# planck-epoch/unet-image-segmentation

Measured on AMD Instinct MI355X. Metric: images/sec (train step, 256x256x3), higher is better.
Workload: dtype f32; 1 GPU; configs[1]: 256x256x3 binary U-Net train step (fwd + dice_loss + bwd + AdamW + MeanIoU(2) update, dropout 0.2); network=U_NET separable-conv, filters 64-128-256-512, bneck 1024, global_batch=16, per_gpu_batch=16, seq_len=65536, parallelism=dp1, batchnorm=per-replica

## Files before the change

unet-image-segmentation_amd/csrc/gemm.h:

```cpp
#pragma once
#include "gemm_plan.h"
#include "view.h"

namespace unet {

struct RowsArgs {
    DView a;
    int64_t M;
    int K;
    int uH, uW, uf;
    const float* B;
    int64_t sbk, sbn;
    int N;
    float* C;
    int64_t ldc;
    const float* bias;
    float2* stats;
    int sH, sW, sf;
    const float* z;
    const float* coef;
    float* side;
    const float *bsc, *bsh, *bmu, *brs;
    float* bnpart;
    float ep_rate, ep_inv_keep;
    uint64_t ep_seed;
    int ko;
    const unsigned short* Bx;
};

struct WgradArgs {
    DView a;
    int P;
    int uH, uW, uf;
    DView b;
    int Q;
    int64_t M, mslice;
    float* slab;
    const float* bz;
    const float* bcoef;
    float* colpart;
};

template <int AMODE, bool DROP, int EPI>
int launch_rows(const RowsArgs& a, hipStream_t st, const char* what);
bool rows_vec_ok(const RowsArgs& a, int amode);
int run_wgrad(WgradArgs a, int amode, int bmode, float* out, void* ws, size_t ws_bytes, hipStream_t st,
              const char* what);
size_t wgrad_workspace(int64_t M, int P, int Q);

inline DView plain_view(const float* p, int c) {
    unet_view v{};
    v.mode = UNET_VIEW_PLAIN;
    v.c0 = c;
    v.src0 = p;
    return make_dview(v);
}
inline bool fits_i32(int64_t a, int64_t b) { return a * b < (int64_t(1) << 31); }
inline int check_planes(const unsigned short* p, const char* what) {
    UNET_CHECK_ARG(p && (uintptr_t)p % 16 == 0, "%s must be a 16-B aligned plane set", what);
    return 0;
}

__device__ __forceinline__ int acc_row(int r, int hi) { return (r & 3) + 8 * (r >> 2) + 4 * hi; }

__device__ __forceinline__ void xcd_group_order(int groups, int sibs, int& grp, int& sib) {
    grp = blockIdx.x;
    sib = blockIdx.y;
    if (sibs > 1 && (groups & 7) == 0) {
        const int L = blockIdx.x + blockIdx.y * groups, u = L >> 3;
        grp = (u / sibs) * 8 + (L & 7);
        sib = u % sibs;
    }
}
__device__ __forceinline__ void xcd_group_order_sx(int sibs, int groups, int& sib, int& grp) {
    sib = blockIdx.x;
    grp = blockIdx.y;
    if (sibs > 1 && (groups & 7) == 0) {
        const int L = blockIdx.x + blockIdx.y * sibs, u = L >> 3;
        grp = (u / sibs) * 8 + (L & 7);
        sib = u % sibs;
    }
}

__device__ __forceinline__ int shuffle_tap_off(int c, int W, int f) {
    const int ab = c / f;
    const int co = c - ab * f;
    return (ab >> 1) * (2 * W * f) + (ab & 1) * f + co;
}


#ifdef UNET_LAB_BUILD
#define ROWS_KO(g, bit) (((g).ko & (bit)) != 0)
__device__ __forceinline__ void lab_stagger(int ko) {
    const int n = (ko >> 8) & 255;
    if (n == 0) return;
    const unsigned lin = blockIdx.x + blockIdx.y * gridDim.x, tot = gridDim.x * gridDim.y;
    const bool late = (ko & 0x10000) ? (lin & 1) : (lin >= tot / 2);
    if (late)
        for (int i = 0; i < n; ++i) __builtin_amdgcn_s_sleep(32);
}
#define ROWS_STAGGER(g) lab_stagger((g).ko)
#define ROWS_STAMP(g, i)                                                                       \
    do {                                                                                       \
        if (((g).ko & 0x20000) && threadIdx.x == 0) {                                          \
            const unsigned lin_ = blockIdx.x + blockIdx.y * gridDim.x;                         \
            if (lin_ < 65536) lab_rows_stamps[4 * lin_ + (i)] =                               \
                ((i) == 0 || (i) == 3) ? __builtin_amdgcn_s_memrealtime() : __builtin_amdgcn_s_memtime(); \
        }                                                                                      \
    } while (0)
#else
#define ROWS_KO(g, bit) false
#define ROWS_STAGGER(g) ((void)0)
#define ROWS_STAMP(g, i) ((void)0)
#endif

}
```

unet-image-segmentation_amd/csrc/gemm_wgrad.hip:

```cpp
#include "dispatch.h"
#include "gemm.h"

namespace unet {
namespace {

template <int BP, int BQ, int AMODE, bool ADROP, int BMODE, bool BDROP>
__global__ __launch_bounds__(256) void gemm_wgrad_kernel(WgradArgs g) {
    constexpr int LDA = BP + 4, LDB = BQ + 4;
    constexpr int TM = BP / 64, TN = BQ / 64;
    constexpr int AR = BP / 16, BR = BQ / 16;
    constexpr int AS = 256 / BP, BS = 256 / BQ;
    __shared__ float As[2][BK][LDA];
    __shared__ float Bs[2][BK][LDB];

    const int tid = threadIdx.x, lane = tid & 63, wave = tid >> 6;
    const int wp = wave >> 1, wq = wave & 1;
    const int lo = lane & 31, hi = lane >> 5;
    const int ntp = (g.P + BP - 1) / BP;
    const int p0 = (blockIdx.x % ntp) * BP;
    const int q0 = (blockIdx.x / ntp) * BQ;
    const int64_t mb = (int64_t)blockIdx.y * g.mslice;
    const int64_t me = mb + g.mslice < g.M ? mb + g.mslice : g.M;

    const int ap = tid % BP, amm = tid / BP;
    const int p = p0 + ap;
    const bool pv = p < g.P;
    float asc = 1.f, ash = 0.f;
    int poff = p;
    if constexpr (AMODE == W_BNRELU) {
        if (pv) {
            asc = g.a.sc0[p];
            ash = g.a.sh0[p];
        }
    }
    if constexpr (AMODE == W_UNSHUFFLE) {
        const int ab = p / g.uf;
        const int co = p - ab * g.uf;
        poff = (ab >> 1) * (2 * g.uW * g.uf) + (ab & 1) * g.uf + co;
    }
    const int bq = tid % BQ, bmm = tid / BQ;
    const int q = q0 + bq;
    const bool qv = q < g.Q;
    float bsc = 1.f, bsh = 0.f;
    if constexpr (BMODE == W_BNRELU) {
        if (qv) {
            bsc = g.b.sc0[q];
            bsh = g.b.sh0[q];
        }
    }

    float ra[AR], rb[BR];
    auto load_stage = [&](int64_t k0) {
#pragma unroll
        for (int r = 0; r < AR; ++r) {
            const int64_t m = k0 + amm + AS * r;
            float v = 0.f;
            if (pv && m < me) {
                if constexpr (AMODE == W_UNSHUFFLE) {
                    const int64_t hw = (int64_t)g.uH * g.uW;
                    const int n = (int)(m / hw);
                    const int rem = (int)(m - n * hw);
                    const int i = rem / g.uW, j = rem - (rem / g.uW) * g.uW;
                    v = g.a.src0[(int64_t)((n * 2 * g.uH + 2 * i) * 2 * g.uW + 2 * j) * g.uf + poff];
                } else {
                    v = g.a.src0[m * g.a.c0 + p];
                    if constexpr (AMODE == W_BNRELU) v = bnrelu(v, asc, ash);
                    if constexpr (ADROP) v *= drop_mult(g.a.seed, (uint64_t)m * g.a.C + p, g.a.rate, g.a.inv_keep);
                }
            }
            ra[r] = v;
        }
#pragma unroll
        for (int r = 0; r < BR; ++r) {
            const int64_t m = k0 + bmm + BS * r;
            float v = 0.f;
            if (qv && m < me) {
                v = g.b.src0[m * g.b.c0 + q];
                if constexpr (BMODE == W_BNRELU) v = bnrelu(v, bsc, bsh);
                if constexpr (BDROP) v *= drop_mult(g.b.seed, (uint64_t)m * g.b.C + q, g.b.rate, g.b.inv_keep);
            }
            rb[r] = v;
        }
    };
    auto store_stage = [&](int buf) {
#pragma unroll
        for (int r = 0; r < AR; ++r) As[buf][amm + AS * r][ap] = ra[r];
#pragma unroll
        for (int r = 0; r < BR; ++r) Bs[buf][bmm + BS * r][bq] = rb[r];
    };

    floatx16 acc[TM][TN];
#pragma unroll
    for (int tm = 0; tm < TM; ++tm)
#pragma unroll
        for (int tn = 0; tn < TN; ++tn)
#pragma unroll
            for (int r = 0; r < 16; ++r) acc[tm][tn][r] = 0.f;

    const int nk = (int)((me - mb + BK - 1) / BK);
    if (nk > 0) {
        load_stage(mb);
        store_stage(0);
    }
    __syncthreads();
    for (int kt = 0; kt < nk; ++kt) {
        const int buf = kt & 1;
        if (kt + 1 < nk) load_stage(mb + (int64_t)(kt + 1) * BK);
#pragma unroll
        for (int kk = 0; kk < BK / 2; ++kk) {
            float av[TM], bv[TN];
#pragma unroll
            for (int tm = 0; tm < TM; ++tm) av[tm] = As[buf][2 * kk + hi][wp * (BP / 2) + tm * 32 + lo];
#pragma unroll
            for (int tn = 0; tn < TN; ++tn) bv[tn] = Bs[buf][2 * kk + hi][wq * (BQ / 2) + tn * 32 + lo];
#pragma unroll
            for (int tm = 0; tm < TM; ++tm)
#pragma unroll
                for (int tn = 0; tn < TN; ++tn)
                    acc[tm][tn] = __builtin_amdgcn_mfma_f32_32x32x2f32(av[tm], bv[tn], acc[tm][tn], 0, 0, 0);
        }
        if (kt + 1 < nk) store_stage(buf ^ 1);
        __syncthreads();
    }
    float* slab = g.slab + (int64_t)blockIdx.y * g.P * g.Q;
#pragma unroll
    for (int tm = 0; tm < TM; ++tm)
#pragma unroll
        for (int tn = 0; tn < TN; ++tn) {
            const int qq = q0 + wq * (BQ / 2) + tn * 32 + lo;
            if (qq >= g.Q) continue;
#pragma unroll
            for (int r = 0; r < 16; ++r) {
                const int pp = p0 + wp * (BP / 2) + tm * 32 + acc_row(r, hi);
                if (pp < g.P) slab[(int64_t)pp * g.Q + qq] = acc[tm][tn][r];
            }
        }
}

template <int BP, int BQ, int AMODE, bool ADROP, int BMODE, bool BDROP>
__global__ __launch_bounds__(256, 1) void gemm_wgrad_vec(WgradArgs g) {
    constexpr int LDA = BP + 4, LDB = BQ + 4;
    constexpr int TM = BP / 64, TN = BQ / 64;
    constexpr int PQ = BP / 4, QQ = BQ / 4;
    constexpr int AR = BK * PQ / 256, BR = BK * QQ / 256;
    constexpr int AS = 256 / PQ, BS = 256 / QQ;
    __shared__ __attribute__((aligned(16))) char smem[4 * 2 * BK * (LDA + LDB)];
    float (*As)[BK * LDA] = reinterpret_cast<float (*)[BK * LDA]>(smem);
    float (*Bs)[BK * LDB] = reinterpret_cast<float (*)[BK * LDB]>(smem + 4 * 2 * BK * LDA);

    const int tid = threadIdx.x, lane = tid & 63, wave = tid >> 6;
    const int wp = wave >> 1, wq = wave & 1;
    const int lo = lane & 31, hi = lane >> 5;
    const int ntp = (g.P + BP - 1) / BP;
    int tile, slice;
    xcd_group_order_sx(gridDim.x, gridDim.y, tile, slice);
    const int p0 = (tile % ntp) * BP;
    const int q0 = (tile / ntp) * BQ;
    const int mb = (int)(slice * g.mslice);
    const int me = (int)((mb + g.mslice) < g.M ? (mb + g.mslice) : g.M);

    const int apq = tid % PQ, amm = tid / PQ;
    const int p = p0 + 4 * apq;
    const bool pv = p < g.P;
    float4 asc = f4(1.f), ash = f4(0.f);
    int poff = p;
    if constexpr (AMODE == W_BNRELU) {
        if (pv) {
            asc = ld4(g.a.sc0 + p);
            ash = ld4(g.a.sh0 + p);
        }
    }
    if constexpr (AMODE == W_UNSHUFFLE) {
        const int ab = p / g.uf;
        const int co = p - ab * g.uf;
        poff = (ab >> 1) * (2 * g.uW * g.uf) + (ab & 1) * g.uf + co;
    }
    const int bqq = tid % QQ, bmm = tid / QQ;
    const int q = q0 + 4 * bqq;
    const bool qv = q < g.Q;
    float4 bsc = f4(1.f), bsh = f4(0.f), bmu = f4(0.f), bp_ = f4(0.f), bq_ = f4(0.f);
    if constexpr (BMODE == W_BNRELU || BMODE == W_BNBWD) {
        if (qv) {
            bsc = ld4(g.b.sc0 + q);
            bsh = ld4(g.b.sh0 + q);
        }
    }
    if constexpr (BMODE == W_BNBWD) {
        if (qv) {
            bmu = ld4(g.bcoef + q);
            bp_ = ld4(g.bcoef + g.Q + q);
            bq_ = ld4(g.bcoef + 2 * g.Q + q);
        }
    }

    float4 ra[AR], rb[BR];
    int ur[AMODE == W_UNSHUFFLE ? AR : 1], uj[AMODE == W_UNSHUFFLE ? AR : 1];
    if constexpr (AMODE == W_UNSHUFFLE) {
#pragma unroll
        for (int r = 0; r < AR; ++r) {
            const int m = mb + amm + AS * r;
            ur[r] = m / g.uW;
            uj[r] = m - ur[r] * g.uW;
        }
    }
    auto load_stage = [&](int k0) {
#pragma unroll
        for (int r = 0; r < AR; ++r) {
            const int m = k0 + amm + AS * r;
            float4 v = f4(0.f);
            if (pv && m < me) {
                if constexpr (AMODE == W_UNSHUFFLE) {
                    v = ld4(g.a.src0 + (4 * ur[r] * g.uW + 2 * uj[r]) * g.uf + poff);
                } else {
                    v = ld4(g.a.src0 + (int64_t)m * g.a.c0 + p);
                    if constexpr (AMODE == W_BNRELU) v = bnrelu4(v, asc, ash);
                    if constexpr (ADROP) {
                        const uint64_t i = (uint64_t)m * g.a.C + p;
                        v = mul4(v, drop_mult4(g.a.seed, i, g.a.rate, g.a.inv_keep));
                    }
                }
            }
            ra[r] = v;
        }
#pragma unroll
        for (int r = 0; r < BR; ++r) {
            const int m = k0 + bmm + BS * r;
            float4 v = f4(0.f);
            if (qv && m < me) {
                v = ld4(g.b.src0 + (int64_t)m * g.b.c0 + q);
                if constexpr (BMODE == W_BNRELU) v = bnrelu4(v, bsc, bsh);
                if constexpr (BMODE == W_BNBWD)
                    bn_bwd_dz4(v, ld4(g.bz + (int64_t)m * g.b.c0 + q), bsc, bsh, bmu, bp_, bq_);
                if constexpr (BDROP) {
                    const uint64_t i = (uint64_t)m * g.b.C + q;
                    v = mul4(v, drop_mult4(g.b.seed, i, g.b.rate, g.b.inv_keep));
                }
            }
            rb[r] = v;
        }
        if constexpr (AMODE == W_UNSHUFFLE) {
#pragma unroll
            for (int r = 0; r < AR; ++r) {
                uj[r] += BK;
                while (uj[r] >= g.uW) {
                    uj[r] -= g.uW;
                    ++ur[r];
                }
            }
        }
    };
    const bool csum_on = g.colpart != nullptr && tile < ntp;
    float4 csum = f4(0.f);
    auto store_stage = [&](int buf) {
#pragma unroll
        for (int r = 0; r < AR; ++r) *reinterpret_cast<float4*>(&As[buf][(amm + AS * r) * LDA + 4 * apq]) = ra[r];
#pragma unroll
        for (int r = 0; r < BR; ++r) *reinterpret_cast<float4*>(&Bs[buf][(bmm + BS * r) * LDB + 4 * bqq]) = rb[r];
        if (csum_on) {
#pragma unroll
            for (int r = 0; r < AR; ++r) csum = add4(csum, ra[r]);
        }
    };

    floatx16 acc[TM][TN];
#pragma unroll
    for (int tm = 0; tm < TM; ++tm)
#pragma unroll
        for (int tn = 0; tn < TN; ++tn)
#pragma unroll
            for (int r = 0; r < 16; ++r) acc[tm][tn][r] = 0.f;

    const int nk = (me - mb + BK - 1) / BK;
    if (nk > 0) {
        load_stage(mb);
        store_stage(0);
    }
    __syncthreads();
    for (int kt = 0; kt < nk; ++kt) {
        const int buf = kt & 1;
        if (kt + 1 < nk) load_stage(mb + (kt + 1) * BK);
#pragma unroll
        for (int kk = 0; kk < BK / 2; ++kk) {
            float av[TM], bv[TN];
#pragma unroll
            for (int tm = 0; tm < TM; ++tm) av[tm] = As[buf][(2 * kk + hi) * LDA + wp * (BP / 2) + tm * 32 + lo];
#pragma unroll
            for (int tn = 0; tn < TN; ++tn) bv[tn] = Bs[buf][(2 * kk + hi) * LDB + wq * (BQ / 2) + tn * 32 + lo];
#pragma unroll
            for (int tm = 0; tm < TM; ++tm)
#pragma unroll
                for (int tn = 0; tn < TN; ++tn)
                    acc[tm][tn] = __builtin_amdgcn_mfma_f32_32x32x2f32(av[tm], bv[tn], acc[tm][tn], 0, 0, 0);
        }
        if (kt + 1 < nk) store_stage(buf ^ 1);
        __syncthreads();
    }
    if (csum_on) {
        float4* T = reinterpret_cast<float4*>(&As[0][0]);
        T[tid] = csum;
        __syncthreads();
        if (tid < PQ && pv) {
            float4 t = T[tid];
            for (int j = 1; j < AS; ++j) t = add4(t, T[j * PQ + tid]);
            st4(g.colpart + (int64_t)slice * g.P + p, t);
        }
    }
    float* slab = g.slab + (int64_t)slice * g.P * g.Q;
#pragma unroll
    for (int tm = 0; tm < TM; ++tm)
#pragma unroll
        for (int tn = 0; tn < TN; ++tn) {
            const int qq = q0 + wq * (BQ / 2) + tn * 32 + lo;
            if (qq >= g.Q) continue;
#pragma unroll
            for (int r = 0; r < 16; ++r) {
                const int pp = p0 + wp * (BP / 2) + tm * 32 + acc_row(r, hi);
                if (pp < g.P) slab[(int64_t)pp * g.Q + qq] = acc[tm][tn][r];
            }
        }
}

template <int AMODE, bool ADROP, int BMODE, bool BDROP>
void launch_wgrad_t(const WgradArgs& a, const WgradPlan& w, hipStream_t st) {
    dim3 grid((unsigned)w.tiles, (unsigned)w.S);
    const unsigned pad = (unsigned)lab_knob("UNET_WGRAD_LDSPAD", 0);
    const bool vec = a.P % 4 == 0 && a.Q % 4 == 0 && (AMODE != W_UNSHUFFLE || a.uf % 4 == 0) &&
                     (AMODE == W_UNSHUFFLE || a.a.c0 % 4 == 0) && a.b.c0 % 4 == 0 &&
                     ((uintptr_t)a.a.src0 | (uintptr_t)a.b.src0) % 16 == 0;
    const bool vk = vec || BMODE == W_BNBWD;
    with_int<128, 64>(w.bp, [&](auto BP) {
        with_int<128, 64>(w.bq, [&](auto BQ) {
            if (vk) gemm_wgrad_vec<BP(), BQ(), AMODE, ADROP, BMODE, BDROP><<<grid, 256, pad, st>>>(a);
            else if constexpr (BMODE != W_BNBWD)
                gemm_wgrad_kernel<BP(), BQ(), AMODE, ADROP, BMODE, BDROP><<<grid, 256, pad, st>>>(a);
        });
    });
}

}

int run_wgrad(WgradArgs a, int amode, int bmode, float* out, void* ws, size_t ws_bytes, hipStream_t st,
              const char* what) {
    WgradPlan w = wgrad_plan(a.M, a.P, a.Q);
    const size_t need = (size_t)w.S * a.P * a.Q * sizeof(float);
    UNET_CHECK_ARG(ws && ws_bytes >= need, "%s: workspace %zu < %zu", what, ws_bytes, need);
    a.mslice = w.mslice;
    a.slab = static_cast<float*>(ws);
    const bool ad = a.a.rate > 0.f, bd = a.b.rate > 0.f;
    if (amode == W_PLAIN && bmode == W_PLAIN) {
        launch_wgrad_t<W_PLAIN, false, W_PLAIN, false>(a, w, st);
    } else if (amode == W_UNSHUFFLE && (bmode == W_BNRELU || bmode == W_PLAIN)) {
        with_int<W_BNRELU, W_PLAIN>(bmode, [&](auto BM) {
            with_bool(bd, [&](auto BD) { launch_wgrad_t<W_UNSHUFFLE, false, BM(), BD()>(a, w, st); });
        });
    } else if (amode == W_BNRELU && bmode == W_PLAIN) {
        with_bool(ad, [&](auto AD) { launch_wgrad_t<W_BNRELU, AD(), W_PLAIN, false>(a, w, st); });
    } else {
        UNET_CHECK_ARG(false, "%s: unsupported wgrad operand modes %d/%d", what, amode, bmode);
    }
    UNET_CHECK_LAUNCH(what);
    return reduce_slabs(a.slab, w.S, (int64_t)a.P * a.Q, out, (int64_t)a.P * a.Q, (int64_t)a.P * a.Q, st);
}

size_t wgrad_workspace(int64_t M, int P, int Q) {
    WgradPlan w = wgrad_plan(M, P, Q);
    return align_up((size_t)w.S * P * Q * sizeof(float), 256);
}

int head_wgrad(const unet_view* x, int64_t M, const float* dlogit, int ncls, float* dkernel, void* ws, size_t ws_bytes,
               hipStream_t st) {
    WgradArgs a{};
    a.a = make_dview(*x);
    a.P = x->c0;
    a.b = plain_view(dlogit, ncls);
    a.Q = ncls;
    a.M = M;
    return run_wgrad(a, x->mode == UNET_VIEW_BNRELU ? W_BNRELU : W_PLAIN, W_PLAIN, dkernel, ws, ws_bytes, st,
                     "unet_head_bwd(filter)");
}
size_t head_wgrad_workspace(int64_t M, int cin, int ncls) { return wgrad_workspace(M, cin, ncls); }

}
```

Before: 1660 images/sec.

## Defer B-side BN-ReLU/dropout to store stage and cut unshuffle index registers in wgrad

For the unshuffle A-mode wgrad kernel with BN-ReLU or dropout on B, the per-channel scale/shift now live in LDS and are applied at store time instead of being held in registers across the loop. The unshuffle row/column tracking is reworked into wave-uniform per-row column counters, and the epilogue indices are recomputed from an opaque copy of tid. These changes aim to lower VGPR pressure in the vec wgrad kernel. One variant also gets extra dynamic LDS padding to cap occupancy at a fixed LDS size, which deliberately limits co-resident blocks.

```diff
diff --git a/unet-image-segmentation_amd/csrc/gemm.h b/unet-image-segmentation_amd/csrc/gemm.h
--- a/unet-image-segmentation_amd/csrc/gemm.h
+++ b/unet-image-segmentation_amd/csrc/gemm.h
@@ -61,6 +61,11 @@
     return 0;
 }
 
+constexpr int kSimdRegs = 512;
+constexpr int kMainSmallRegs = 80;
+constexpr int kMainSmallLds = 16384;
+constexpr unsigned kSideCap3Lds = 45056;
+
 __device__ __forceinline__ int acc_row(int r, int hi) { return (r & 3) + 8 * (r >> 2) + 4 * hi; }
 
 __device__ __forceinline__ void xcd_group_order(int groups, int sibs, int& grp, int& sib) {
diff --git a/unet-image-segmentation_amd/csrc/gemm_wgrad.hip b/unet-image-segmentation_amd/csrc/gemm_wgrad.hip
--- a/unet-image-segmentation_amd/csrc/gemm_wgrad.hip
+++ b/unet-image-segmentation_amd/csrc/gemm_wgrad.hip
@@ -144,9 +144,12 @@
     constexpr int PQ = BP / 4, QQ = BQ / 4;
     constexpr int AR = BK * PQ / 256, BR = BK * QQ / 256;
     constexpr int AS = 256 / PQ, BS = 256 / QQ;
-    __shared__ __attribute__((aligned(16))) char smem[4 * 2 * BK * (LDA + LDB)];
+    constexpr bool LATEB = AMODE == W_UNSHUFFLE && (BMODE == W_BNRELU || BDROP);
+    constexpr int STAGE_BYTES = 4 * 2 * BK * (LDA + LDB);
+    __shared__ __attribute__((aligned(16))) char smem[STAGE_BYTES + (LATEB ? 8 * BQ : 0)];
     float (*As)[BK * LDA] = reinterpret_cast<float (*)[BK * LDA]>(smem);
     float (*Bs)[BK * LDB] = reinterpret_cast<float (*)[BK * LDB]>(smem + 4 * 2 * BK * LDA);
+    float* bview = reinterpret_cast<float*>(smem + (LATEB ? STAGE_BYTES : 0));
 
     const int tid = threadIdx.x, lane = tid & 63, wave = tid >> 6;
     const int wp = wave >> 1, wq = wave & 1;
@@ -179,11 +182,19 @@
     const int q = q0 + 4 * bqq;
     const bool qv = q < g.Q;
     float4 bsc = f4(1.f), bsh = f4(0.f), bmu = f4(0.f), bp_ = f4(0.f), bq_ = f4(0.f);
-    if constexpr (BMODE == W_BNRELU || BMODE == W_BNBWD) {
+    if constexpr ((BMODE == W_BNRELU || BMODE == W_BNBWD) && !LATEB) {
         if (qv) {
             bsc = ld4(g.b.sc0 + q);
             bsh = ld4(g.b.sh0 + q);
         }
+    }
+    if constexpr (LATEB && BMODE == W_BNRELU) {
+        if (tid < BQ) {
+            const bool v = q0 + tid < g.Q;
+            bview[tid] = v ? g.b.sc0[q0 + tid] : 1.f;
+            bview[BQ + tid] = v ? g.b.sh0[q0 + tid] : 0.f;
+        }
+        __syncthreads();
     }
     if constexpr (BMODE == W_BNBWD) {
         if (qv) {
@@ -194,14 +205,15 @@
     }
 
     float4 ra[AR], rb[BR];
-    int ur[AMODE == W_UNSHUFFLE ? AR : 1], uj[AMODE == W_UNSHUFFLE ? AR : 1];
+    constexpr int RW = 64 / PQ;
+    const int wrow = __builtin_amdgcn_readfirstlane(wave) * RW;
+    const int asub = amm - wrow;
+    int uj[AMODE == W_UNSHUFFLE ? AR : 1][RW];
     if constexpr (AMODE == W_UNSHUFFLE) {
 #pragma unroll
-        for (int r = 0; r < AR; ++r) {
-            const int m = mb + amm + AS * r;
-            ur[r] = m / g.uW;
-            uj[r] = m - ur[r] * g.uW;
-        }
+        for (int r = 0; r < AR; ++r)
+#pragma unroll
+            for (int k = 0; k < RW; ++k) uj[r][k] = (mb + wrow + AS * r + k) % g.uW;
     }
     auto load_stage = [&](int k0) {
 #pragma unroll
@@ -210,7 +222,10 @@
             float4 v = f4(0.f);
             if (pv && m < me) {
                 if constexpr (AMODE == W_UNSHUFFLE) {
-                    v = ld4(g.a.src0 + (4 * ur[r] * g.uW + 2 * uj[r]) * g.uf + poff);
+                    int off = (4 * (k0 + wrow + AS * r) - 2 * uj[r][0]) * g.uf;
+#pragma unroll
+                    for (int k = 1; k < RW; ++k) off = asub == k ? (4 * (k0 + wrow + AS * r + k) - 2 * uj[r][k]) * g.uf : off;
+                    v = ld4(g.a.src0 + off + poff);
                 } else {
                     v = ld4(g.a.src0 + (int64_t)m * g.a.c0 + p);
                     if constexpr (AMODE == W_BNRELU) v = bnrelu4(v, asc, ash);
@@ -228,32 +243,52 @@
             float4 v = f4(0.f);
             if (qv && m < me) {
                 v = ld4(g.b.src0 + (int64_t)m * g.b.c0 + q);
-                if constexpr (BMODE == W_BNRELU) v = bnrelu4(v, bsc, bsh);
+                if constexpr (BMODE == W_BNRELU && !LATEB) v = bnrelu4(v, bsc, bsh);
                 if constexpr (BMODE == W_BNBWD)
                     bn_bwd_dz4(v, ld4(g.bz + (int64_t)m * g.b.c0 + q), bsc, bsh, bmu, bp_, bq_);
+                if constexpr (BDROP && !LATEB) {
+                    const uint64_t i = (uint64_t)m * g.b.C + q;
+                    v = mul4(v, drop_mult4(g.b.seed, i, g.b.rate, g.b.inv_keep));
+                }
+            }
+            rb[r] = v;
+        }
+        if constexpr (AMODE == W_UNSHUFFLE) {
+#pragma unroll
+            for (int r = 0; r < AR; ++r)
+#pragma unroll
+                for (int k = 0; k < RW; ++k) {
+                    uj[r][k] += BK;
+                    while (uj[r][k] >= g.uW) uj[r][k] -= g.uW;
+                }
+        }
+    };
+    const bool csum_on = g.colpart != nullptr && tile < ntp;
+    float4 csum = f4(0.f);
+    auto store_stage = [&](int buf, int k0) {
+#pragma unroll
+        for (int r = 0; r < AR; ++r) *reinterpret_cast<float4*>(&As[buf][(amm + AS * r) * LDA + 4 * apq]) = ra[r];
+        if constexpr (LATEB) {
+            float4 sc = f4(1.f), sh = f4(0.f);
+            if constexpr (BMODE == W_BNRELU) {
+                unsigned t = tid;
+                asm volatile("" : "+v"(t));
+                const float4* tv = reinterpret_cast<const float4*>(bview) + t % QQ;
+                sc = tv[0];
+                sh = tv[QQ];
+            }
+#pragma unroll
+            for (int r = 0; r < BR; ++r) {
+                const int m = k0 + bmm + BS * r;
+                float4 v = rb[r];
+                if constexpr (BMODE == W_BNRELU) v = bnrelu4(v, sc, sh);
                 if constexpr (BDROP) {
                     const uint64_t i = (uint64_t)m * g.b.C + q;
                     v = mul4(v, drop_mult4(g.b.seed, i, g.b.rate, g.b.inv_keep));
                 }
-            }
-            rb[r] = v;
-        }
-        if constexpr (AMODE == W_UNSHUFFLE) {
-#pragma unroll
-            for (int r = 0; r < AR; ++r) {
-                uj[r] += BK;
-                while (uj[r] >= g.uW) {
-                    uj[r] -= g.uW;
-                    ++ur[r];
-                }
-            }
-        }
-    };
-    const bool csum_on = g.colpart != nullptr && tile < ntp;
-    float4 csum = f4(0.f);
-    auto store_stage = [&](int buf) {
-#pragma unroll
-        for (int r = 0; r < AR; ++r) *reinterpret_cast<float4*>(&As[buf][(amm + AS * r) * LDA + 4 * apq]) = ra[r];
+                rb[r] = qv && m < me ? v : f4(0.f);
+            }
+        }
 #pragma unroll
         for (int r = 0; r < BR; ++r) *reinterpret_cast<float4*>(&Bs[buf][(bmm + BS * r) * LDB + 4 * bqq]) = rb[r];
         if (csum_on) {
@@ -273,7 +308,7 @@
     const int nk = (me - mb + BK - 1) / BK;
     if (nk > 0) {
         load_stage(mb);
-        store_stage(0);
+        store_stage(0, mb);
     }
     __syncthreads();
     for (int kt = 0; kt < nk; ++kt) {
@@ -292,17 +327,23 @@
                 for (int tn = 0; tn < TN; ++tn)
                     acc[tm][tn] = __builtin_amdgcn_mfma_f32_32x32x2f32(av[tm], bv[tn], acc[tm][tn], 0, 0, 0);
         }
-        if (kt + 1 < nk) store_stage(buf ^ 1);
+        if (kt + 1 < nk) store_stage(buf ^ 1, mb + (kt + 1) * BK);
         __syncthreads();
+    }
+    int et = tid, elo = lo, ehi = hi, ewp = wp, ewq = wq, ep = p;
+    if constexpr (AMODE == W_UNSHUFFLE) {
+        asm volatile("" : "+v"(et));
+        elo = et & 31, ehi = (et >> 5) & 1, ewp = et >> 7, ewq = (et >> 6) & 1;
+        ep = p0 + 4 * (et % PQ);
     }
     if (csum_on) {
         float4* T = reinterpret_cast<float4*>(&As[0][0]);
-        T[tid] = csum;
+        T[et] = csum;
         __syncthreads();
-        if (tid < PQ && pv) {
-            float4 t = T[tid];
-            for (int j = 1; j < AS; ++j) t = add4(t, T[j * PQ + tid]);
-            st4(g.colpart + (int64_t)slice * g.P + p, t);
+        if (et < PQ && ep < g.P) {
+            float4 t = T[et];
+            for (int j = 1; j < AS; ++j) t = add4(t, T[j * PQ + et]);
+            st4(g.colpart + (int64_t)slice * g.P + ep, t);
         }
     }
     float* slab = g.slab + (int64_t)slice * g.P * g.Q;
@@ -310,11 +351,11 @@
     for (int tm = 0; tm < TM; ++tm)
 #pragma unroll
         for (int tn = 0; tn < TN; ++tn) {
-            const int qq = q0 + wq * (BQ / 2) + tn * 32 + lo;
+            const int qq = q0 + ewq * (BQ / 2) + tn * 32 + elo;
             if (qq >= g.Q) continue;
 #pragma unroll
             for (int r = 0; r < 16; ++r) {
-                const int pp = p0 + wp * (BP / 2) + tm * 32 + acc_row(r, hi);
+                const int pp = p0 + ewp * (BP / 2) + tm * 32 + acc_row(r, ehi);
                 if (pp < g.P) slab[(int64_t)pp * g.Q + qq] = acc[tm][tn][r];
             }
         }
@@ -330,7 +371,10 @@
     const bool vk = vec || BMODE == W_BNBWD;
     with_int<128, 64>(w.bp, [&](auto BP) {
         with_int<128, 64>(w.bq, [&](auto BQ) {
-            if (vk) gemm_wgrad_vec<BP(), BQ(), AMODE, ADROP, BMODE, BDROP><<<grid, 256, pad, st>>>(a);
+            constexpr bool cap3 = AMODE == W_UNSHUFFLE && BMODE == W_BNRELU && BDROP && BP() == 128 && BQ() == 128;
+            constexpr unsigned lds = 4 * 2 * BK * (BP() + BQ() + 8) + 8 * BQ();
+            if (vk) gemm_wgrad_vec<BP(), BQ(), AMODE, ADROP, BMODE, BDROP>
+                    <<<grid, 256, cap3 ? kSideCap3Lds - lds + pad : pad, st>>>(a);
             else if constexpr (BMODE != W_BNBWD)
                 gemm_wgrad_kernel<BP(), BQ(), AMODE, ADROP, BMODE, BDROP><<<grid, 256, pad, st>>>(a);
         });
```

Result: slower. 1639 images/sec (-1.3%).
